# SuperbTUM/real-time-ReID-tracking

Hardware: AMD Instinct MI355X
Metric: crops/sec embedded + NxM distmat ms, ResNet18-SE 128x256 (higher is better)
Workload: dtype f16x3; 1 GPU; BASELINE configs[1]: ResNet18-SE embed 4096 distinct uint8 crops (128x256) per GPU + 4096x4096 L2 distmat; crops_per_gpu=4096, embed_dim=512, chunk=1024

## Files before the change

real-time-reid-tracking_amd/csrc/debug.hip:

```cpp
#include "reid_internal.h"
#include "pil_launch.h"
#include <string.h>
#include <stdlib.h>
#include <vector>

namespace {
struct Switch { const char* name; int reid_ctx::* field; };
const Switch kSwitches[] = {
    {"f16_cfg", &reid_ctx::f16_cfg}, {"f16_lin_256", &reid_ctx::f16_lin_256}, {"f16_split_k", &reid_ctx::f16_split_k},
    {"bank_fast", &reid_ctx::bank_fast}, {"side_copy", &reid_ctx::side_copy}, {"f32_stem_pool", &reid_ctx::f32_stem_pool},
    {"stem_split", &reid_ctx::stem_split}, {"split_pair", &reid_ctx::split_pair}, {"split_lean_epi", &reid_ctx::split_lean_epi},
    {"knn_wide", &reid_ctx::knn_wide}, {"f16_loader_prio", &reid_ctx::f16_loader_prio}, {"f16_frag_ahead", &reid_ctx::f16_frag_ahead},
    {"pack_epilogue", &reid_ctx::pack_epilogue}, {"f16_wide_splitk", &reid_ctx::f16_wide_splitk}, {"f32_split_k", &reid_ctx::f32_split_k},
    {"swin_fold", &reid_ctx::swin_fold}, {"swin_stop", &reid_ctx::swin_stop}, {"select_two_pass", &reid_ctx::select_two_pass},
    {"split_terms", &reid_ctx::split_terms}, {"f32_conv", &reid_ctx::f32_conv}, {"swin_attn_mfma", &reid_ctx::swin_attn_mfma},
    {"swin_attn_split", &reid_ctx::swin_attn_split}, {"swin_two_linear", &reid_ctx::swin_two_linear},
    {"f16_loader_waves", &reid_ctx::f16_loader_waves}, {"f16_halo", &reid_ctx::f16_halo}, {"f16_stem_fused", &reid_ctx::f16_stem_fused},
    {"f16_se_tail", &reid_ctx::f16_se_tail}, {"f16_c64", &reid_ctx::f16_c64}, {"swin_chunk_cap", &reid_ctx::swin_chunk_cap},
    {"split_x3", &reid_ctx::split_x3}, {"x3_ablate", &reid_ctx::x3_ablate}, {"x3_unroll", &reid_ctx::x3_unroll}, {"x3_narrow", &reid_ctx::x3_narrow}, {"conv_x3s", &reid_ctx::conv_x3s}, {"x3s_sk_cap", &reid_ctx::x3s_sk_cap}, {"x3_l4_narrow_nmt", &reid_ctx::x3_l4_narrow_nmt}, {"split_x3_small", &reid_ctx::split_x3_small}, {"split_x3_min_blocks", &reid_ctx::split_x3_min_blocks}, {"f32_dist_bk16", &reid_ctx::f32_dist_bk16}, {"lin_x3", &reid_ctx::lin_x3},
    {"host_pipeline", &reid_ctx::host_pipeline}, {"x3_sk_cap", &reid_ctx::x3_sk_cap}, {"chain", &reid_ctx::chain}, {"split_gemm_min_tiles", &reid_ctx::split_gemm_min_tiles},
    {"rerank_hbm_acc", &reid_ctx::rerank_hbm_acc}, {"gem_tail_min", &reid_ctx::gem_tail_min}, {"anysize_force", &reid_ctx::anysize_force},
};
}

extern "C" int reid_debug_set_switch(reid_ctx* ctx, const char* name, long long value) {
    ARG_CHECK(ctx && name);
    CTX_GUARD(ctx);
    HIP_TRY(hipStreamSynchronize(ctx->stream));
    if (!strcmp(name, "knn_wide_min")) {
        ctx->knn_wide_min = value;
        return REID_OK;
    }
    for (const Switch& s : kSwitches)
        if (!strcmp(name, s.name)) {
            if (!strcmp(name, "split_terms") && value != 3 && value != 4) break;
            ctx->*(s.field) = (int)value;
            return REID_OK;
        }
    reid_set_error("reid_debug_set_switch: no switch '%s' (or a value it does not take)", name);
    return REID_ERR_ARG;
}

extern "C" int reid_debug_get_switch(reid_ctx* ctx, const char* name, long long* value) {
    ARG_CHECK(ctx && name && value);
    if (!strcmp(name, "knn_wide_min")) {
        *value = ctx->knn_wide_min;
        return REID_OK;
    }
    for (const Switch& s : kSwitches)
        if (!strcmp(name, s.name)) {
            *value = ctx->*(s.field);
            return REID_OK;
        }
    reid_set_error("reid_debug_get_switch: no switch '%s'", name);
    return REID_ERR_ARG;
}

extern "C" int reid_debug_conv_f16(reid_ctx* ctx, int n, int h, int w, int cin, int cout, int r, int stride, int pad, int cfg,
                                   int iters, float* ms_per_launch) {
    ARG_CHECK(ctx && ms_per_launch && ctx->se18.loaded);
    CTX_GUARD(ctx);
    typedef _Float16 f16;
    const int ho = (h + 2 * pad - r) / stride + 1, wo = (w + 2 * pad - r) / stride + 1;
    const size_t nin = (size_t)n * h * w * cin, nw = (size_t)cout * r * r * cin, nout = (size_t)n * ho * wo * cout;
    f16 *x, *wt, *out;
    REID_TRY(ctx_ws(ctx, "dbg.x", nin * 2, (void**)&x));
    REID_TRY(ctx_ws(ctx, "dbg.w", nw * 2, (void**)&wt));
    REID_TRY(ctx_ws(ctx, "dbg.out", nout * 2, (void**)&out));
    const size_t src_n = ctx->se18.n_floats;
    for (size_t o = 0; o < nin; o += src_n) REID_TRY(launch_f32_to_f16(ctx, ctx->se18.blob, nin - o < src_n ? nin - o : src_n, x + o));
    for (size_t o = 0; o < nw; o += src_n) REID_TRY(launch_f32_to_f16(ctx, ctx->se18.blob, nw - o < src_n ? nw - o : src_n, wt + o));
    if (getenv("REID_DEBUG_ZERO")) {
        HIP_TRY(hipMemsetAsync(x, 0, nin * 2, ctx->stream));
        HIP_TRY(hipMemsetAsync(wt, 0, nw * 2, ctx->stream));
    }
    const int c0 = ctx->f16_cfg;
    const int h0 = ctx->f16_halo;
    ctx->f16_halo = cfg >= 2000000 ? 2 : 0;
    const int l0 = ctx->f16_loader_waves;
    if (cfg >= 2000000) ctx->f16_loader_waves = cfg & 1;
    ctx->f16_cfg = cfg >= 2000000 ? 0 : cfg;
    int st = REID_OK;
    for (int i = 0; i < 2 && st == REID_OK; ++i)
        st = conv_gemm16(ctx, A16_IM2COL, x, n, h, w, cin, wt, cout, r, r, stride, pad, r * r * cin, nullptr, nullptr, nullptr, 0, nullptr, out);
    if (st == REID_OK) st = reid_timer_start(ctx);
    for (int i = 0; i < iters && st == REID_OK; ++i)
        st = conv_gemm16(ctx, A16_IM2COL, x, n, h, w, cin, wt, cout, r, r, stride, pad, r * r * cin, nullptr, nullptr, nullptr, 0, nullptr, out);
    float ms = 0.f;
    if (st == REID_OK) st = reid_timer_stop(ctx, &ms);
    ctx->f16_cfg = c0;
    ctx->f16_halo = h0;
    ctx->f16_loader_waves = l0;
    *ms_per_launch = ms / (iters > 0 ? iters : 1);
    return st;
}


extern "C" int reid_debug_conv_split(reid_ctx* ctx, int n, int h, int w, int c, int cout, int ablate, int iters, float* ms_per_launch) {
    ARG_CHECK(ctx && ms_per_launch && ctx->se18.loaded && c % 64 == 0 && cout % 64 == 0);
    CTX_GUARD(ctx);
    typedef _Float16 f16;
    const size_t nin = (size_t)n * h * w * 2 * c, nw = (size_t)cout * 9 * 3 * c, nout = (size_t)n * h * w * cout;
    f16 *x, *wt;
    float *out, *sc;
    REID_TRY(ctx_ws(ctx, "dbgs.x", nin * 2, (void**)&x));
    REID_TRY(ctx_ws(ctx, "dbgs.w", nw * 2, (void**)&wt));
    REID_TRY(ctx_ws(ctx, "dbgs.out", nout * 4, (void**)&out));
    REID_TRY(ctx_ws(ctx, "dbgs.sc", (size_t)cout * 2 * 4, (void**)&sc));
    const size_t src_n = ctx->se18.n_floats;
    for (size_t o = 0; o < nin; o += src_n) REID_TRY(launch_f32_to_f16(ctx, ctx->se18.blob, nin - o < src_n ? nin - o : src_n, x + o));
    for (size_t o = 0; o < nw; o += src_n) REID_TRY(launch_f32_to_f16(ctx, ctx->se18.blob, nw - o < src_n ? nw - o : src_n, wt + o));
    HIP_TRY(hipMemcpyAsync(sc, ctx->se18.blob, (size_t)cout * 2 * 4, hipMemcpyDeviceToDevice, ctx->stream));
    if (ablate & 128) {
        HIP_TRY(hipMemsetAsync(x, 0, nin * 2, ctx->stream));
        HIP_TRY(hipMemsetAsync(wt, 0, nw * 2, ctx->stream));
    }
    Gemm16Params q;
    memset(&q, 0, sizeof(q));
    q.split_terms = 3;
    q.H = h; q.W = w; q.Cin = 3 * c; q.R = 3; q.S = 3; q.stride = 1; q.pad = 1; q.Ho = h; q.Wo = w;
    q.M = n * h * w; q.N = cout; q.K = 27 * c; q.ldb = q.K;
    q.A = x; q.B = wt; q.C32 = out; q.ldc = cout;
    q.col_scale = sc; q.col_shift = sc + cout; q.relu = 1;
    q.acc_scale = 1.0f / 2048.0f;
    q.zero_page = ctx->se18.zero_page;
    q.ablate = ablate & 127;
    q.diag = ctx->conv_diag;
    int st = REID_OK;
    for (int i = 0; i < 2 && st == REID_OK; ++i) st = launch_conv3x3_split(ctx, q, REID_K_CONV_GEMM, 0, 0);
    if (st == REID_OK) st = reid_timer_start(ctx);
    for (int i = 0; i < iters && st == REID_OK; ++i) st = launch_conv3x3_split(ctx, q, REID_K_CONV_GEMM, 0, 0);
    float ms = 0.f;
    if (st == REID_OK) st = reid_timer_stop(ctx, &ms);
    *ms_per_launch = ms / (iters > 0 ? iters : 1);
    return st;
}

extern "C" int reid_debug_conv_c64(reid_ctx* ctx, int n, const float* x, const float* w_krsc, const float* scale,
                                   const float* shift, const float* residual, int relu, float* out, float* stats) {
    ARG_CHECK(ctx && x && w_krsc && out && n >= 1);
    CTX_GUARD(ctx);
    typedef _Float16 f16;
    const size_t nact = (size_t)n * 64 * 32 * 64, nw = 64 * 576;
    float *xf, *wf, *rf = nullptr, *sc = nullptr, *sh = nullptr, *st = nullptr, *of;
    f16 *xh, *wh, *rh = nullptr, *oh, *zp;
    REID_TRY(ctx_ws(ctx, "dbg64.xf", nact * 4, (void**)&xf));
    REID_TRY(ctx_ws(ctx, "dbg64.wf", nw * 4, (void**)&wf));
    REID_TRY(ctx_ws(ctx, "dbg64.xh", nact * 2, (void**)&xh));
    REID_TRY(ctx_ws(ctx, "dbg64.wh", nw * 2, (void**)&wh));
    REID_TRY(ctx_ws(ctx, "dbg64.oh", nact * 2, (void**)&oh));
    REID_TRY(ctx_ws(ctx, "dbg64.of", nact * 4, (void**)&of));
    REID_TRY(ctx_ws(ctx, "dbg64.zp", 256, (void**)&zp));
    REID_TRY(ctx_ws(ctx, "dbg64.sc", 64 * 4, (void**)&sc));
    REID_TRY(ctx_ws(ctx, "dbg64.sh", 64 * 4, (void**)&sh));
    REID_TRY(ctx_ws(ctx, "dbg64.st", (size_t)n * 128 * 4, (void**)&st));
    HIP_TRY(hipMemsetAsync(zp, 0, 256, ctx->stream));
    HIP_TRY(hipMemcpyAsync(xf, x, nact * 4, hipMemcpyHostToDevice, ctx->stream));
    HIP_TRY(hipMemcpyAsync(wf, w_krsc, nw * 4, hipMemcpyHostToDevice, ctx->stream));
    std::vector<float> ones(64, 1.f);
    HIP_TRY(hipMemcpyAsync(sc, scale ? scale : ones.data(), 64 * 4, hipMemcpyHostToDevice, ctx->stream));
    if (shift) HIP_TRY(hipMemcpyAsync(sh, shift, 64 * 4, hipMemcpyHostToDevice, ctx->stream));
    REID_TRY(launch_f32_to_f16(ctx, xf, nact, xh));
    REID_TRY(launch_scale_rows_f16(ctx, wf, sc, 64, 576, wh));
    if (residual) {
        REID_TRY(ctx_ws(ctx, "dbg64.rf", nact * 4, (void**)&rf));
        REID_TRY(ctx_ws(ctx, "dbg64.rh", nact * 2, (void**)&rh));
        HIP_TRY(hipMemcpyAsync(rf, residual, nact * 4, hipMemcpyHostToDevice, ctx->stream));
        REID_TRY(launch_f32_to_f16(ctx, rf, nact, rh));
    }
    HIP_TRY(hipStreamSynchronize(ctx->stream));
    REID_TRY(launch_conv3x3_c64_f16(ctx, xh, n, wh, shift ? sh : nullptr, rh, relu, stats ? st : nullptr, oh, zp));
    std::vector<f16> tmp(nact);
    HIP_TRY(hipMemcpyAsync(tmp.data(), oh, nact * 2, hipMemcpyDeviceToHost, ctx->stream));
    if (stats) HIP_TRY(hipMemcpyAsync(stats, st, (size_t)n * 128 * 4, hipMemcpyDeviceToHost, ctx->stream));
// ... 1253 lines not shown
```

real-time-reid-tracking_amd/csrc/reid_internal.h:

```cpp
#pragma once
#include <hip/hip_runtime.h>
#include <stdint.h>
#include <stddef.h>
#include <stdio.h>
#include <initializer_list>
#include <string>
#include <map>
#include <tuple>
#include <vector>
#include "../../include/reid_hip.h"
struct reid_ctx;

void reid_set_error(const char* fmt, ...);

#define HIP_TRY(expr)                                                                         \
    do {                                                                                      \
        hipError_t _e = (expr);                                                               \
        if (_e != hipSuccess) {                                                               \
            reid_set_error("%s:%d %s -> %s", __FILE__, __LINE__, #expr, hipGetErrorString(_e)); \
            return REID_ERR_HIP;                                                              \
        }                                                                                     \
    } while (0)

#define REID_TRY(expr)            \
// ... 202 lines not shown
int launch_scale_rows_f16(reid_ctx*, const float* w, const float* scale, int rows, int k, _Float16* out);
int launch_conv3x3_c64_f16(reid_ctx*, const _Float16* in, int n, const _Float16* w_scaled, const float* shift,
                           const _Float16* residual, int relu, float* stats, _Float16* out, const _Float16* zero_page,
                           const float* se_w1 = nullptr, const float* se_w2t = nullptr);
int launch_stem_w16_scaled(reid_ctx*, const float* stem_w_f32, const float* scale, _Float16* out);
int launch_stem_pool_f16(reid_ctx*, const _Float16* pad_in, const uint8_t* crops_u8, int n, const _Float16* w16s, const float* shift,
                         _Float16* pooled);
int launch_conv_w16_chunked(reid_ctx*, const float* w_f32, int cout, int rs, int cin, _Float16* out);
int launch_gemm_f32(reid_ctx* ctx, int amode, int epi, const GemmParams& p, int kind, double flops, double bytes);
int launch_ta_tail(reid_ctx* ctx, const float* y, const float* sc, int n_img, int H, int W, int C, const float* wts, float* out);
int launch_ema_tail(reid_ctx* ctx, const float* y, const float* sc, int n_img, int H, int W, int C, const float* prm, float* out);
int launch_stem_split(reid_ctx* ctx, const void* x, bool is_u8, int n, const float* wgt, const float* scale, const float* shift, float* out,
                      _Float16* packed);
int launch_stem_f32(reid_ctx* ctx, const void* x, bool is_u8, int n, const float* wgt, const float* scale, const float* shift,
                    float* out, bool pooled);
bool gemm_f32_dma_supported(int amode, int epi, const GemmParams& p);
int launch_gemm_f32_dma(reid_ctx* ctx, int epi, const GemmParams& p, int kind, double flops, double bytes);
bool conv_f32_supported(const GemmParams& p);
int launch_conv_f32(reid_ctx* ctx, const GemmParams& p, int kind, double flops, double bytes);
bool conv_f32_general_supported(const GemmParams& p);
int launch_conv_f32_general(reid_ctx* ctx, const GemmParams& p, int kind, double flops, double bytes);

int launch_nchw_to_nhwc3(reid_ctx*, const float* x_nchw, int n, int h, int w, float* out_nhwc);
int launch_resize_norm(reid_ctx*, const uint8_t* packed, const long long* offsets, const int* hw, int n, int H, int W,
                       int pitch, float* out_nhwc);
int launch_maxpool3s2(reid_ctx*, const float* x, int n, int h, int w, int c, float* out);
int launch_norm_finalize(reid_ctx*, const float* stats, int n_img, int tiles, int c, int half, int hw,
                         const float* in_gamma, const float* in_beta, const float* bn_scale, const float* bn_shift,
                         float* a_scale, float* a_shift);
int launch_in_apply(reid_ctx*, float* x, const float* stats, int n_img, int tiles, int c, int half, int hw, const float* in_gamma,
                    const float* in_beta);
int launch_se_finalize(reid_ctx*, const float* stats, int n_img, int tiles, int c, int mid, int hw, const float* w1,
                       const float* w2, float* s);
int tail_slices(int n_img, int hw);
int launch_se_tail(reid_ctx*, const float* stats, int n_img, int tiles, int c, int mid, int hw, const float* w1, const float* w2,
                   const float* y, const float* sc, float* out, _Float16* packed = nullptr);
int launch_se_tail_form(reid_ctx*, int form, const float* stats, int n_img, int tiles, int c, int mid, int hw, const float* w1,
                        const float* w2, const float* y, const float* sc, float* out, _Float16* packed);
int launch_se_combine(reid_ctx*, const float* y, const float* sc, const float* s, int n_img, int hw, int c, float* out);
int launch_in_apply_pack(reid_ctx*, const float* x, const float* stats, int n_img, int tiles, int c, int half, int hw,
                         const float* in_gamma, const float* in_beta, _Float16* packed,
                         bool in_half_only = false);
int launch_gem_neck(reid_ctx*, const float* x, int n_img, int hw, int c, const float* p, const float* scale,
                    const float* shift, float* gem_out, float* emb);
int launch_gem_neck_tail(reid_ctx*, const float* stats, int n_img, int tiles, int c, int mid, int hw, const float* w1, const float* w2,
                         const float* y, const float* sc, const float* p, const float* scale, const float* shift, float* gem_out,
                         float* emb);
int launch_row_sqnorm(reid_ctx*, const float* x, int m, int d, long long ld, float* out);
int launch_argmin_rows(reid_ctx*, const float* dist, int m, int n, long long ld, int32_t* idx, float* val);
int launch_topk_rows(reid_ctx*, const float* dist, int m, int n, long long ld, int k, float* D, int32_t* I);
int launch_rank_eval(reid_ctx*, const float* score, int nq, int ng, long long ld, const long long* ql,
                     const long long* qc, const long long* gl, const long long* gc, int32_t* cmc_sum, double* ap,
                     int32_t* valid);
int launch_diou_cost(reid_ctx*, const double* tracks, int t, const double* dets, int m, double* out, int as_cost);

struct ProfSlot {
    double ms = 0, flops = 0, bytes = 0;
    long long launches = 0;
};

struct Se18Block {
    int c, cin, stride, ibn, ds, mid;
    const float *conv1_w, *in_gamma, *in_beta, *bn1_scale, *bn1_shift, *conv2_w, *bn2_scale, *bn2_shift;
    const float *ds_w, *ds_scale, *ds_shift, *se_w1, *se_w2;
    const float *ta, *ema;
};

struct Se18Weights {
    bool loaded = false;
    float* blob = nullptr;
    size_t n_floats = 0;
    int num_class = 0;
    int arch = 0;
    const float *stem_w, *stem_scale, *stem_shift;
    Se18Block blk[8];
    const float *gem_p, *neck_scale, *neck_shift, *cls_w;
    const float* cam_bias = nullptr;
    int num_cams = 0;
    float cam_factor = -1.0f;
    _Float16* blob16 = nullptr;
    _Float16* stem_w16 = nullptr;
    _Float16* l1_conv2_w16s[2] = {nullptr, nullptr};
    _Float16* stem_w16s = nullptr;
    _Float16* zero_page = nullptr;
    float* ep = nullptr;
    const _Float16* h(const float* p) const { return blob16 + (p - blob); }
};

struct reid_comm_loop {
    virtual int allgather(int rank, const void* d_send, void* d_recv, size_t bytes, hipStream_t st) = 0;
    virtual int allreduce(int rank, double* inout, int count, int op) = 0;
    virtual void detach(int rank) = 0;
    virtual ~reid_comm_loop() {}
};
struct reid_comm {
    void* comm = nullptr;
    int rank = 0, world = 1;
    reid_comm_loop* loop = nullptr;
};
void comm_release(reid_ctx* ctx);
int launch_knn_merge(reid_ctx* ctx, const float* Dall, const int32_t* Iall, int world, int nq, int kk, int k, float* D, int32_t* I);

struct reid_ctx {
    int device = 0;
    reid_comm* comm = nullptr;
    hipStream_t stream = nullptr;
    hipStream_t own_stream = nullptr;
    int chunk = 1024;
    int precision = 0;
    bool profile = false;
    ProfSlot prof[REID_K_COUNT];
    std::vector<std::pair<hipEvent_t, hipEvent_t>> ev_pool;
    struct Pending { int kind; hipEvent_t a, b; double flops, bytes; };
    std::vector<Pending> pending;
    hipEvent_t t0 = nullptr, t1 = nullptr;
    std::map<std::string, std::pair<void*, size_t>> ws;
    std::map<std::string, std::pair<void*, size_t>> pinned;
    std::map<const void*, void*> split_w;
    int bank_fast = 1;
    Se18Weights se18;
    int last_n = 0;
    int swin_last_n = 0, swin_last_tok = 0;
    int debug_keep = 0;
    bool last_f16 = false;
    int f16_wide_splitk = 1;
    int f16_frag_ahead = 1;
    int f16_loader_prio = 1;
    int f16_loader_waves = 1;
    int f16_halo = 1;
    int gem_tail_min = 120;
    int f16_se_tail = 1;
    int f16_c64 = 2;
    int f16_stem_fused = 2;
    int f32_conv = 1;
    int f32_split_k = 1;
    int lin_x3 = 1;
    int f32_dist_bk16 = 1;
    int pack_epilogue = 1;
    int split_lean_epi = 1;
    int split_x3 = 3;
    int split_gemm_min_tiles = 128;
    int chain = 0;
    int x3_sk_cap = 0;
    int split_x3_small = 2;
    int x3s_sk_cap = 8;
    int conv_x3s = 1;
    int x3_l4_narrow_nmt = 31;
    int x3_narrow = 1;
    int x3_unroll = 3;
    int x3_ablate = 0;
    int split_x3_min_blocks = 512;
    int split_pair = 0;
    int stem_split = 1;
    int f32_stem_pool = 1;
    int split_terms = 3;
    int knn_wide = 1;
    long long knn_wide_min = 1ll << 25;
    int knn_wide_force = 0;
    int select_exp = 0;
    int select_two_pass = 0;
    int rerank_hbm_acc = 0;
    int swin_stop = -1;
    int swin_fold = 1;
    int swin_two_linear = 1;
    int swin_attn_split = 0;
    int two_linear_ablate = 0;
    int swin_attn_mfma = 1;
    int f16_split_k = 1;
    int swin_chunk_cap = 1024;
    int f16_lin_256 = 1;
    int f16_cfg = 0;
    int frame_m[2] = {0, 0};
    float* frame_emb[2] = {nullptr, nullptr};
    int frame_d[2] = {512, 512};
    int frame_pending[2] = {0, 0}, frame_has[2] = {0, 0};
    size_t frame_tm[2] = {0, 0};
    hipEvent_t frame_ev[2] = {nullptr, nullptr};
    hipStream_t match_stream = nullptr;
    int match_async = 0;
    hipEvent_t join_ev = nullptr;
    hipEvent_t fwd_ev[2] = {nullptr, nullptr}, match_ev[2] = {nullptr, nullptr};
    hipStream_t copy_stream = nullptr;
    hipEvent_t copy_ev = nullptr;
    std::vector<hipEvent_t> pipe_ev;
    int host_pipeline = 1;
    int side_copy = 1;
    std::vector<int32_t> side_idx;
    size_t side_cursor = 0;
    const char* frame_out[2] = {nullptr, nullptr};
    float* stage_ptr[11] = {nullptr};
    size_t stage_elems[11] = {0};
    int anysize_force = 0;
    unsigned long long* conv_diag = nullptr;
    int conv_form = 0;
    std::string split_bad_se18, split_bad_swin;
    int* fault = nullptr;
};
enum { REID_FAULT_RANGE = 1, REID_FAULT_NONFINITE = 2 };
int ctx_fault_status(reid_ctx* ctx);
bool knn_wide_eligible(reid_ctx* ctx, int nq, int nb, int d, int k);
int knn_wide_dev(reid_ctx* ctx, const float* xp, int nq, const float* yp, int nb, int ld, const float* rs, const float* cq, int k, float* d_D,
                 int32_t* d_I);

inline std::string split_range_violation(const float* blob, const std::map<std::string, std::pair<size_t, size_t>>& tab,
                                         const std::vector<std::pair<std::string, float>>& suffix_bound) {
    for (const auto& kv : tab) {
        for (const auto& sb : suffix_bound) {
            const std::string& suf = sb.first;
            if (kv.first.size() < suf.size() || kv.first.compare(kv.first.size() - suf.size(), suf.size(), suf) != 0) continue;
            float mx = 0.f;
            const float* w = blob + kv.second.first;
            for (size_t i = 0; i < kv.second.second; ++i) {
                const float a = w[i] < 0 ? -w[i] : w[i];
                if (!(a <= mx)) mx = a;
            }
            if (!(mx < sb.second)) {
                char buf[160];
                snprintf(buf, sizeof(buf), "%s (max |w| = %g, limit %g)", kv.first.c_str(), (double)mx, (double)sb.second);
                return buf;
            }
            break;
        }
    }
    return std::string();
}

struct ChainElem {
    const float* x;
    const float* stats;
    const float* sc;
    const float *g, *b;
    float* out;
    _Float16* packed;
    int c, half, hw, tiles, mid, slices;
};
struct ChainStage {
    int kind;
    int idx;
    int first, items;
    int dep;
    int target;
    int sk;
};
struct ChainParams {
    int n_img, n_stages, total_items, flags;
    ChainStage st[8];
    Gemm16Params conv[4];
    ChainElem el[4];
    int* counters;
    int* fault;
};
int launch_chain(reid_ctx* ctx, const ChainParams& cp, int W);

int conv_gemm(reid_ctx* ctx, int amode, const void* x, int n, int H, int W, int Cin, const float* wgt, int Cout, int R,
              int S, int stride, int pad, int Kpad, const float* a_scale, const float* a_shift, int a_relu,
              const float* col_scale, const float* col_shift, const float* residual, int relu, float* stats, float* out,
              int relu_from = 0, const _Float16* x_packed = nullptr,
              _Float16* out_packed = nullptr, int pack_from = 0, bool* packed_written = nullptr);
int conv_weights_fresh(reid_ctx* ctx, const float* d_w);
int conv_weights_splittable(reid_ctx* ctx, const float* h_w, size_t count, const char* who);
int conv_gemm16(reid_ctx* ctx, int amode, const _Float16* x, int n, int H, int W, int Cin, const _Float16* wgt, int Cout,
                int R, int S, int stride, int pad, int K, const float* col_scale, const float* col_shift,
                const _Float16* residual, int relu, float* stats, _Float16* out, int Hp = 0, int Wp = 0);

struct DeviceGuard {
    int prev = -1, dev = -1;
    explicit DeviceGuard(int d) : dev(d) {
        if (hipGetDevice(&prev) != hipSuccess) prev = -1;
        if (prev != dev) (void)hipSetDevice(dev);
    }
    ~DeviceGuard() {
        if (prev >= 0 && prev != dev) (void)hipSetDevice(prev);
    }
    DeviceGuard(const DeviceGuard&) = delete;
    DeviceGuard& operator=(const DeviceGuard&) = delete;
};
#define CTX_GUARD(ctx) DeviceGuard _dev_guard((ctx)->device)
#define CTX_ENTER(ctx)            \
    CTX_GUARD(ctx);               \
    REID_TRY(ctx_fault_status(ctx))

void swin_release(reid_ctx* ctx);
int ctx_ws(reid_ctx* ctx, const char* name, size_t bytes, void** out);
int ctx_take_side(reid_ctx* ctx, int n, int rows, const char* what, const int32_t** d_idx);
int launch_add_indexed_rows(reid_ctx* ctx, float* x, int n, long long hw, int C, const float* table, const int32_t* d_idx, float coeff);
int ctx_pinned(reid_ctx* ctx, const char* name, size_t bytes, void** out);
int ctx_pipe_events(reid_ctx* ctx, int passes);

template <class Up, class Run, class Down>
int host_passes(reid_ctx* ctx, int n, int pass, Up up, Run run, Down down) {
    const int passes = (n + pass - 1) / pass;
    if (passes <= 1 || !ctx->host_pipeline) {
        REID_TRY(up(0, n, ctx->stream));
        for (int i = 0; i < n; i += pass) REID_TRY(run(i, n - i < pass ? n - i : pass));
        REID_TRY(down(0, n, ctx->stream));
        HIP_TRY(hipStreamSynchronize(ctx->stream));
        return REID_OK;
    }
    REID_TRY(ctx_pipe_events(ctx, passes));
    hipStream_t cs = ctx->copy_stream;
    hipEvent_t* up_ev = ctx->pipe_ev.data();
    hipEvent_t* run_ev = ctx->pipe_ev.data() + passes;
    auto span = [&](int k, int* i, int* m) { *i = k * pass; *m = n - *i < pass ? n - *i : pass; };
    int i, m, rc = REID_OK;
    span(0, &i, &m);
    rc = up(i, m, cs);
// ... 111 lines not shown
```

real-time-reid-tracking_amd/csrc/stem_split.hip:

```cpp
#include "reid_internal.h"

typedef _Float16 f16;
typedef f16 half8 __attribute__((ext_vector_type(8)));
typedef float f32x16 __attribute__((ext_vector_type(16)));
typedef unsigned int u32x2 __attribute__((ext_vector_type(2)));

namespace {

constexpr int IMG_H = 256, IMG_W = 128, OUT_H = 128, OUT_W = 64;
constexpr int PITCH = 144 * 8;
constexpr int RING = 32;
constexpr int WROW = 14 * 32 + 16;

__device__ __forceinline__ unsigned split_pair(float x) {
    const f16 h = (f16)x;
    const f16 l = (f16)((x - (float)h) * 2048.0f);
    return (unsigned)__builtin_bit_cast(unsigned short, h) | ((unsigned)__builtin_bit_cast(unsigned short, l) << 16);
}

template <bool U8>
__global__ __launch_bounds__(512, 1) void stem_split_kernel(const void* __restrict__ x, const float* __restrict__ wgt,
                                                            const float* __restrict__ scale, const float* __restrict__ shift,
                                                            int nseg, float* __restrict__ out, f16* __restrict__ packed,
                                                            int* __restrict__ fault) {
    extern __shared__ __attribute__((aligned(16))) unsigned char smem[];
    unsigned char* const img_h = smem;
    unsigned char* const img_l = img_h + RING * PITCH;
    unsigned char* const w_h = img_l + RING * PITCH;
    unsigned char* const w_l = w_h + 64 * WROW;
    float* const edge = (float*)(w_l + 64 * WROW);

    const int tid = threadIdx.x, lane = tid & 63, wave = tid >> 6;
    const int li = lane & 31, lh = lane >> 5;
    const int cw = wave & 3, cb = wave >> 2;
    const int img = blockIdx.x / nseg, seg = blockIdx.x - img * nseg;
    const int t0 = seg * (OUT_H / 2) / nseg, t1 = (seg + 1) * (OUT_H / 2) / nseg;

    for (int i = tid; i < 2 * RING * PITCH / 16; i += 512) ((uint4*)smem)[i] = uint4{0u, 0u, 0u, 0u};
    __syncthreads();
    for (int i = tid; i < 64 * 14 * 16; i += 512) {
        const int n = i / 224, k = i - n * 224, s = k >> 4, h = (k >> 3) & 1, j = k & 7;
        const int px = 2 * (2 * (s & 1) + h) + (j >> 2), c = j & 3;
        const float v = (px < 7 && c < 3) ? wgt[n * 192 + (s >> 1) * 24 + px * 3 + c] : 0.f;
        const unsigned hl = split_pair(v);
        *(unsigned short*)(w_h + n * WROW + k * 2) = (unsigned short)hl;
        *(unsigned short*)(w_l + n * WROW + k * 2) = (unsigned short)(hl >> 16);
        if constexpr (U8) {
            const float wh = (float)__builtin_bit_cast(f16, (unsigned short)hl), wl = (float)__builtin_bit_cast(f16, (unsigned short)(hl >> 16));
            const f16 ll = (f16)(((v - wh) * 2048.0f - wl) * 2048.0f);
            *(unsigned short*)(img_l + n * WROW + k * 2) = __builtin_bit_cast(unsigned short, ll);
        }
    }
    __syncthreads();

    const int f_row = tid >> 7, f_px = tid & 127;
    const int f_off = (3 * f_px) & ~3, f_off2 = f_off + 4 < IMG_W * 3 ? f_off + 4 : f_off, f_sh = 8 * ((3 * f_px) & 3);
    auto fetch = [&](int j, unsigned (&raw)[3]) __attribute__((always_inline)) {
        const int iy = 4 * j + 2 + f_row;
        raw[0] = raw[1] = raw[2] = 0u;
        if ((unsigned)iy < (unsigned)IMG_H) {
            if constexpr (U8) {
                const uint8_t* p = (const uint8_t*)x + ((long long)img * IMG_H + iy) * (IMG_W * 3);
                raw[0] = *(const unsigned*)(p + f_off);
                raw[1] = *(const unsigned*)(p + f_off2);
            } else {
                const float* p = (const float*)x + (((long long)img * IMG_H + iy) * IMG_W + f_px) * 3;
                raw[0] = __float_as_uint(p[0]); raw[1] = __float_as_uint(p[1]); raw[2] = __float_as_uint(p[2]);
            }
        }
    };
    auto commit = [&](int j, const unsigned (&raw)[3]) __attribute__((always_inline)) {
        const int iy = 4 * j + 2 + f_row;
        unsigned a = 0u, b = 0u, c = 0u;
        const int at = ((iy - 2) & (RING - 1)) * PITCH + (3 + f_px) * 8;
        if constexpr (U8) {
            if ((unsigned)iy < (unsigned)IMG_H) {
                const unsigned px = (unsigned)((((unsigned long long)raw[1] << 32) | raw[0]) >> f_sh);
                a = __builtin_bit_cast(unsigned short, (f16)(float)(2 * (int)(px & 0xffu) - 255));
                b = __builtin_bit_cast(unsigned short, (f16)(float)(2 * (int)((px >> 8) & 0xffu) - 255));
                c = __builtin_bit_cast(unsigned short, (f16)(float)(2 * (int)((px >> 16) & 0xffu) - 255));
            }
            *(u32x2*)(img_h + at) = u32x2{a | (b << 16), c};
            return;
        }
        if ((unsigned)iy < (unsigned)IMG_H) {
            a = split_pair(__uint_as_float(raw[0])); b = split_pair(__uint_as_float(raw[1])); c = split_pair(__uint_as_float(raw[2]));
        }
        *(u32x2*)(img_h + at) = u32x2{(a & 0xffffu) | (b << 16), c & 0xffffu};
        *(u32x2*)(img_l + at) = u32x2{(a >> 16) | (b & 0xffff0000u), c >> 16};
    };

    const int ox = cw * 16 + (li & 15);
    const int a_col = (2 * ox + 2 * lh) * 8;
    const int b_at = (cb * 32 + li) * WROW + lh * 16;
    const float cs = U8 ? scale[cb * 32 + li] / 255.0f : scale[cb * 32 + li], sh = shift[cb * 32 + li];

    const int t_first = t0 > 0 ? t0 - 1 : t0;
    const int ntile = t1 - t_first;
    float prev[8], pend = 0.f;
#pragma unroll
    for (int e = 0; e < 8; ++e) prev[e] = -INFINITY;
    float* const pool_img = out + (long long)img * (OUT_H / 2) * (OUT_W / 2) * 64;
    f16* const pack_img = packed ? packed + (long long)img * (OUT_H / 2) * (OUT_W / 2) * 128 : nullptr;
    unsigned vmag = 0u;
    auto store = [&](int t, int col, float v) __attribute__((always_inline)) {
        const long long pix = (long long)t * (OUT_W / 2) + col;
        pool_img[pix * 64 + cb * 32 + li] = v;
        if (pack_img) {
            vmag = range_acc(vmag, v);
            const unsigned hl = split_pair(v);
            *(unsigned short*)(pack_img + pix * 128 + cb * 32 + li) = (unsigned short)hl;
            *(unsigned short*)(pack_img + pix * 128 + 64 + cb * 32 + li) = (unsigned short)(hl >> 16);
        }
    };
    auto finish_first_column = [&](int t) __attribute__((always_inline)) {
        if (cw > 0 && lh == 0) store(t, cw * 8, fmaxf(pend, edge[((t & 1) * 4 + cw - 1) * 64 + cb * 32 + li]));
    };

    unsigned raw_a[3], raw_b[3];
    for (int j = t_first - 2; j <= t_first + 1; ++j) {
        fetch(j, raw_a);
        commit(j, raw_a);
    }
    const int t_last = t_first + ntile - 1;
    fetch(t_first + 2, raw_a);
    __syncthreads();
    auto mma = [&](int t) __attribute__((always_inline)) -> f32x16 {
        f32x16 acc, cor, cor2;
#pragma unroll
        for (int e = 0; e < 16; ++e) acc[e] = cor[e] = cor2[e] = 0.f;
        const int row0 = 4 * t - 5 + 2 * (li >> 4);
        half8 av[3], alv[3], bhv[3], blv[3];
        auto load_step = [&](int st, int buf) __attribute__((always_inline)) {
            const int a_at = ((row0 + (st >> 1)) & (RING - 1)) * PITCH + a_col + 32 * (st & 1);
            av[buf] = *(const half8*)(img_h + a_at);
            bhv[buf] = *(const half8*)(w_h + b_at + 32 * st);
            blv[buf] = *(const half8*)(w_l + b_at + 32 * st);
            if constexpr (U8) alv[buf] = *(const half8*)(img_l + b_at + 32 * st);
            else alv[buf] = *(const half8*)(img_l + a_at);
        };
        load_step(0, 0);
        load_step(1, 1);
#pragma unroll
        for (int st = 0; st < 14; ++st) {
            const int buf = st % 3;
            if (st + 2 < 14) load_step(st + 2, (st + 2) % 3);
            __builtin_amdgcn_sched_barrier(0);
            acc = __builtin_amdgcn_mfma_f32_32x32x16_f16(av[buf], bhv[buf], acc, 0, 0, 0);
            if constexpr (U8) cor2 = __builtin_amdgcn_mfma_f32_32x32x16_f16(av[buf], alv[buf], cor2, 0, 0, 0);
            else cor = __builtin_amdgcn_mfma_f32_32x32x16_f16(alv[buf], bhv[buf], cor, 0, 0, 0);
            cor = __builtin_amdgcn_mfma_f32_32x32x16_f16(av[buf], blv[buf], cor, 0, 0, 0);
            __builtin_amdgcn_sched_barrier(0);
        }
        constexpr float S1 = 1.0f / 2048.0f;
        f32x16 v;
#pragma unroll
        for (int e = 0; e < 16; ++e) v[e] = (acc[e] + (cor[e] + cor2[e] * S1) * S1) * cs + sh;
        return v;
    };
    auto epilogue = [&](int t, const f32x16 v) __attribute__((always_inline)) {
        const bool emit = t >= t0;
        if (emit && t > t_first && t > t0) finish_first_column(t - 1);
        float vm[8];
#pragma unroll
        for (int e = 0; e < 8; ++e) {
            vm[e] = fmaxf(fmaxf(prev[e], v[e]), v[e + 8]);
            prev[e] = v[e + 8];
        }
        if (emit) {
            const float m01 = fmaxf(vm[0], vm[1]), m45 = fmaxf(vm[4], vm[5]);
            const float pa = fmaxf(fmaxf(vm[1], vm[2]), vm[3]), pb = fmaxf(fmaxf(vm[5], vm[6]), vm[7]);
            const float s0 = lh ? m01 : vm[3], s1 = lh ? vm[3] : m45, s2 = lh ? m45 : vm[7];
            const float p2 = fmaxf(s0, __shfl_xor(s0, 32)), p4 = fmaxf(s1, __shfl_xor(s1, 32)), p6 = fmaxf(s2, __shfl_xor(s2, 32));
            store(t, cw * 8 + 1 + 2 * lh, pa);
            store(t, cw * 8 + 5 + 2 * lh, pb);
            store(t, cw * 8 + (lh ? 4 : 2), lh ? p4 : p2);
            if (lh) {
                store(t, cw * 8 + 6, p6);
                edge[((t & 1) * 4 + cw) * 64 + cb * 32 + li] = vm[7];
            } else if (cw == 0) {
                store(t, 0, m01);
            } else {
                pend = m01;
            }
        }
    };
    const bool defer = cb == 1;
    f32x16 vkeep;
#pragma unroll
    for (int e = 0; e < 16; ++e) vkeep[e] = 0.f;
    auto tile = [&](int t, unsigned (&raw_commit)[3], unsigned (&raw_fetch)[3]) __attribute__((always_inline)) {
        if (t + 3 <= t_last) fetch(t + 3, raw_fetch);
        if (defer) {
            if (t > t_first) epilogue(t - 1, vkeep);
            vkeep = mma(t);
        } else {
            vkeep = mma(t);
        }
        if (t + 2 <= t_last) commit(t + 2, raw_commit);
        if (!defer) epilogue(t, vkeep);
        __syncthreads();
    };
    for (int t = t_first; t <= t_last; t += 2) {
        tile(t, raw_a, raw_b);
        if (t + 1 <= t_last) tile(t + 1, raw_b, raw_a);
    }
    if (defer) epilogue(t_last, vkeep);
    __syncthreads();
    finish_first_column(t1 - 1);
    range_raise(fault, vmag);
}

constexpr int SMEM = 2 * RING * PITCH + 2 * 64 * WROW + 2 * 4 * 64 * 4;

}

int launch_stem_split(reid_ctx* ctx, const void* x, bool is_u8, int n, const float* wgt, const float* scale, const float* shift, float* out,
                      _Float16* packed) {
    ARG_CHECK(n >= 1);
    int nseg = 1;
    if (n < 256) {
        long long best = -1;
        for (int s = 1; s <= 64; ++s) {
            const long long rounds = ((long long)n * s + 255) / 256;
            const long long cost = rounds * (3 + 5 * ((64 + s - 1) / s + (s > 1 ? 1 : 0)));
            if (best < 0 || cost < best) { best = cost; nseg = s; }
        }
    }
    const int grid = n * nseg;
    if (is_u8) HIP_TRY(hipFuncSetAttribute((const void*)stem_split_kernel<true>, hipFuncAttributeMaxDynamicSharedMemorySize, SMEM));
    else HIP_TRY(hipFuncSetAttribute((const void*)stem_split_kernel<false>, hipFuncAttributeMaxDynamicSharedMemorySize, SMEM));
    const double flops = 2.0 * n * OUT_H * OUT_W * 64 * 147.0;
    const double bytes = (double)n * IMG_H * IMG_W * 3 * (is_u8 ? 1.0 : 4.0) + (double)n * OUT_H * OUT_W * 64 * (packed ? 2.0 : 1.0) + 64 * 147 * 4.0;
    prof_begin(ctx, REID_K_CONV_GEMM, flops, bytes);
    if (is_u8) hipLaunchKernelGGL((stem_split_kernel<true>), dim3(grid), dim3(512), SMEM, ctx->stream, x, wgt, scale, shift, nseg, out, packed,
                                  ctx->fault);
    else hipLaunchKernelGGL((stem_split_kernel<false>), dim3(grid), dim3(512), SMEM, ctx->stream, x, wgt, scale, shift, nseg, out, packed, ctx->fault);
    prof_end(ctx);
    LAUNCH_CHECK();
    return REID_OK;
}
```

Baseline: 85240 crops/s.

## Make stem conv kernel persistent, walking images per block with prefetch overlap

For large batches the stem conv+pool kernel now launches one block per compute unit, and each block loops over images with a grid stride instead of using one block per image. The first rows of the next image are prefetched while the current image's epilogue finishes, and weight staging into shared memory is paid once per block rather than once per image. The epilogue is also restructured to use precomputed byte offsets and permlane32_swap in place of shuffles, and the wave index is made uniform with readfirstlane. The risk is load imbalance when the image count does not divide evenly by the CU count, and the loss of overlap between independent blocks.

```diff
diff --git a/real-time-reid-tracking_amd/csrc/debug.hip b/real-time-reid-tracking_amd/csrc/debug.hip
--- a/real-time-reid-tracking_amd/csrc/debug.hip
+++ b/real-time-reid-tracking_amd/csrc/debug.hip
@@ -20,6 +20,7 @@
     {"split_x3", &reid_ctx::split_x3}, {"x3_ablate", &reid_ctx::x3_ablate}, {"x3_unroll", &reid_ctx::x3_unroll}, {"x3_narrow", &reid_ctx::x3_narrow}, {"conv_x3s", &reid_ctx::conv_x3s}, {"x3s_sk_cap", &reid_ctx::x3s_sk_cap}, {"x3_l4_narrow_nmt", &reid_ctx::x3_l4_narrow_nmt}, {"split_x3_small", &reid_ctx::split_x3_small}, {"split_x3_min_blocks", &reid_ctx::split_x3_min_blocks}, {"f32_dist_bk16", &reid_ctx::f32_dist_bk16}, {"lin_x3", &reid_ctx::lin_x3},
     {"host_pipeline", &reid_ctx::host_pipeline}, {"x3_sk_cap", &reid_ctx::x3_sk_cap}, {"chain", &reid_ctx::chain}, {"split_gemm_min_tiles", &reid_ctx::split_gemm_min_tiles},
     {"rerank_hbm_acc", &reid_ctx::rerank_hbm_acc}, {"gem_tail_min", &reid_ctx::gem_tail_min}, {"anysize_force", &reid_ctx::anysize_force},
+    {"stem_walk_min", &reid_ctx::stem_walk_min}, {"stem_walk_blocks", &reid_ctx::stem_walk_blocks},
 };
 }
 
diff --git a/real-time-reid-tracking_amd/csrc/reid_internal.h b/real-time-reid-tracking_amd/csrc/reid_internal.h
--- a/real-time-reid-tracking_amd/csrc/reid_internal.h
+++ b/real-time-reid-tracking_amd/csrc/reid_internal.h
@@ -378,6 +378,8 @@
     int split_x3_min_blocks = 512;
     int split_pair = 0;
     int stem_split = 1;
+    int stem_walk_min = 256;
+    int stem_walk_blocks = 0;
     int f32_stem_pool = 1;
     int split_terms = 3;
     int knn_wide = 1;
diff --git a/real-time-reid-tracking_amd/csrc/stem_split.hip b/real-time-reid-tracking_amd/csrc/stem_split.hip
--- a/real-time-reid-tracking_amd/csrc/stem_split.hip
+++ b/real-time-reid-tracking_amd/csrc/stem_split.hip
@@ -30,11 +30,15 @@
     unsigned char* const w_l = w_h + 64 * WROW;
     float* const edge = (float*)(w_l + 64 * WROW);
 
-    const int tid = threadIdx.x, lane = tid & 63, wave = tid >> 6;
+    const int tid = threadIdx.x, lane = tid & 63, wave = __builtin_amdgcn_readfirstlane(tid >> 6);
     const int li = lane & 31, lh = lane >> 5;
     const int cw = wave & 3, cb = wave >> 2;
-    const int img = blockIdx.x / nseg, seg = blockIdx.x - img * nseg;
-    const int t0 = seg * (OUT_H / 2) / nseg, t1 = (seg + 1) * (OUT_H / 2) / nseg;
+    const bool walk = nseg < 0;
+    int img = walk ? (int)blockIdx.x : (int)blockIdx.x / nseg;
+    const int img_end = walk ? -nseg : img + 1, img_step = walk ? (int)gridDim.x : 1;
+    const int seg = walk ? 0 : (int)blockIdx.x - img * nseg, nstrip = walk ? 1 : nseg;
+    const int t0 = seg * (OUT_H / 2) / nstrip, t1 = (seg + 1) * (OUT_H / 2) / nstrip;
+    if (img >= img_end) return;
 
     for (int i = tid; i < 2 * RING * PITCH / 16; i += 512) ((uint4*)smem)[i] = uint4{0u, 0u, 0u, 0u};
     __syncthreads();
@@ -98,33 +102,34 @@
     const int t_first = t0 > 0 ? t0 - 1 : t0;
     const int ntile = t1 - t_first;
     float prev[8], pend = 0.f;
-#pragma unroll
-    for (int e = 0; e < 8; ++e) prev[e] = -INFINITY;
-    float* const pool_img = out + (long long)img * (OUT_H / 2) * (OUT_W / 2) * 64;
-    f16* const pack_img = packed ? packed + (long long)img * (OUT_H / 2) * (OUT_W / 2) * 128 : nullptr;
+    char *pool_img = nullptr, *pack_img = nullptr;
+    const unsigned ch = cb * 32 + li;
+    const unsigned col_a = cw * 8 + 1 + 2 * lh, col_c = cw * 8 + (lh ? 4 : 2), col_d = cw * 8 + (lh ? 6 : 0);
+    const unsigned o32_a = col_a * 256 + ch * 4, o32_c = col_c * 256 + ch * 4, o32_d = col_d * 256 + ch * 4;
+    const unsigned o16_a = col_a * 256 + ch * 2, o16_c = col_c * 256 + ch * 2, o16_d = col_d * 256 + ch * 2;
+    float* const edge_w = edge + cw * 64 + ch;
+    const float* const edge_r = edge + (cw > 0 ? cw - 1 : 0) * 64 + ch;
     unsigned vmag = 0u;
-    auto store = [&](int t, int col, float v) __attribute__((always_inline)) {
-        const long long pix = (long long)t * (OUT_W / 2) + col;
-        pool_img[pix * 64 + cb * 32 + li] = v;
+    auto put = [&](int t, unsigned o32, unsigned o16, int add, float v) __attribute__((always_inline)) {
+        *(float*)(pool_img + (size_t)t * 8192 + add + (size_t)o32) = v;
         if (pack_img) {
             vmag = range_acc(vmag, v);
             const unsigned hl = split_pair(v);
-            *(unsigned short*)(pack_img + pix * 128 + cb * 32 + li) = (unsigned short)hl;
-            *(unsigned short*)(pack_img + pix * 128 + 64 + cb * 32 + li) = (unsigned short)(hl >> 16);
-        }
-    };
-    auto finish_first_column = [&](int t) __attribute__((always_inline)) {
-        if (cw > 0 && lh == 0) store(t, cw * 8, fmaxf(pend, edge[((t & 1) * 4 + cw - 1) * 64 + cb * 32 + li]));
-    };
-
-    unsigned raw_a[3], raw_b[3];
-    for (int j = t_first - 2; j <= t_first + 1; ++j) {
-        fetch(j, raw_a);
-        commit(j, raw_a);
-    }
+            char* const p = pack_img + (size_t)t * 8192 + add + (size_t)o16;
+            *(unsigned short*)p = (unsigned short)hl;
+            *(unsigned short*)(p + 128) = (unsigned short)(hl >> 16);
+        }
+    };
+    auto finish_fourth = [&](int t) __attribute__((always_inline)) {
+        if (cw > 0) put(t, o32_d, o16_d, 0, lh ? pend : fmaxf(pend, edge_r[(t & 1) * 256]));
+    };
+
+    unsigned raw_a[3], raw_b[3], raw4[4][3];
     const int t_last = t_first + ntile - 1;
-    fetch(t_first + 2, raw_a);
-    __syncthreads();
+    auto fetch4 = [&]() __attribute__((always_inline)) {
+#pragma unroll
+        for (int k = 0; k < 4; ++k) fetch(t_first - 2 + k, raw4[k]);
+    };
     auto mma = [&](int t) __attribute__((always_inline)) -> f32x16 {
         f32x16 acc, cor, cor2;
 #pragma unroll
@@ -159,31 +164,27 @@
         return v;
     };
     auto epilogue = [&](int t, const f32x16 v) __attribute__((always_inline)) {
-        const bool emit = t >= t0;
-        if (emit && t > t_first && t > t0) finish_first_column(t - 1);
+        if (t > t0 && t > t_first) finish_fourth(t - 1);
         float vm[8];
 #pragma unroll
         for (int e = 0; e < 8; ++e) {
             vm[e] = fmaxf(fmaxf(prev[e], v[e]), v[e + 8]);
             prev[e] = v[e + 8];
         }
-        if (emit) {
-            const float m01 = fmaxf(vm[0], vm[1]), m45 = fmaxf(vm[4], vm[5]);
-            const float pa = fmaxf(fmaxf(vm[1], vm[2]), vm[3]), pb = fmaxf(fmaxf(vm[5], vm[6]), vm[7]);
-            const float s0 = lh ? m01 : vm[3], s1 = lh ? vm[3] : m45, s2 = lh ? m45 : vm[7];
-            const float p2 = fmaxf(s0, __shfl_xor(s0, 32)), p4 = fmaxf(s1, __shfl_xor(s1, 32)), p6 = fmaxf(s2, __shfl_xor(s2, 32));
-            store(t, cw * 8 + 1 + 2 * lh, pa);
-            store(t, cw * 8 + 5 + 2 * lh, pb);
-            store(t, cw * 8 + (lh ? 4 : 2), lh ? p4 : p2);
-            if (lh) {
-                store(t, cw * 8 + 6, p6);
-                edge[((t & 1) * 4 + cw) * 64 + cb * 32 + li] = vm[7];
-            } else if (cw == 0) {
-                store(t, 0, m01);
-            } else {
-                pend = m01;
-            }
-        }
+        if (t < t0) return;
+        const float m01 = fmaxf(vm[0], vm[1]), m45 = fmaxf(vm[4], vm[5]);
+        const float pa = fmaxf(fmaxf(vm[1], vm[2]), vm[3]), pb = fmaxf(fmaxf(vm[5], vm[6]), vm[7]);
+        const auto x0 = __builtin_amdgcn_permlane32_swap(__float_as_uint(m01), __float_as_uint(m45), false, false);
+        const auto x1 = __builtin_amdgcn_permlane32_swap(__float_as_uint(vm[7]), __float_as_uint(vm[7]), false, false);
+        const float p24 = fmaxf(vm[3], __uint_as_float(lh ? x0[0] : x0[1]));
+        const float p6 = fmaxf(m45, __uint_as_float(x1[0]));
+        put(t, o32_a, o16_a, 0, pa);
+        put(t, o32_a, o16_a, 4 * 256, pb);
+        put(t, o32_c, o16_c, 0, p24);
+        if (lh) edge_w[(t & 1) * 256] = vm[7];
+        const float fourth = lh ? p6 : m01;
+        if (cw == 0) put(t, o32_d, o16_d, 0, fourth);
+        else pend = fourth;
     };
     const bool defer = cb == 1;
     f32x16 vkeep;
@@ -201,13 +202,28 @@
         if (!defer) epilogue(t, vkeep);
         __syncthreads();
     };
-    for (int t = t_first; t <= t_last; t += 2) {
-        tile(t, raw_a, raw_b);
-        if (t + 1 <= t_last) tile(t + 1, raw_b, raw_a);
-    }
-    if (defer) epilogue(t_last, vkeep);
-    __syncthreads();
-    finish_first_column(t1 - 1);
+    fetch4();
+    for (;;) {
+#pragma unroll
+        for (int k = 0; k < 4; ++k) commit(t_first - 2 + k, raw4[k]);
+        fetch(t_first + 2, raw_a);
+        pool_img = (char*)out + (size_t)img * ((OUT_H / 2) * (OUT_W / 2) * 64 * 4);
+        pack_img = packed ? (char*)packed + (size_t)img * ((OUT_H / 2) * (OUT_W / 2) * 128 * 2) : nullptr;
+#pragma unroll
+        for (int e = 0; e < 8; ++e) prev[e] = -INFINITY;
+        __syncthreads();
+        for (int t = t_first; t <= t_last; t += 2) {
+            tile(t, raw_a, raw_b);
+            if (t + 1 <= t_last) tile(t + 1, raw_b, raw_a);
+        }
+        img += img_step;
+        const bool more = img < img_end;
+        if (more) fetch4();
+        if (defer) epilogue(t_last, vkeep);
+        __syncthreads();
+        finish_fourth(t1 - 1);
+        if (!more) break;
+    }
     range_raise(fault, vmag);
 }
 
@@ -227,7 +243,13 @@
             if (best < 0 || cost < best) { best = cost; nseg = s; }
         }
     }
-    const int grid = n * nseg;
+    int grid = n * nseg;
+    if (n >= ctx->stem_walk_min) {
+        int blocks = ctx->stem_walk_blocks;
+        if (blocks <= 0) HIP_TRY(hipDeviceGetAttribute(&blocks, hipDeviceAttributeMultiprocessorCount, ctx->device));
+        grid = n < blocks ? n : blocks;
+        nseg = -n;
+    }
     if (is_u8) HIP_TRY(hipFuncSetAttribute((const void*)stem_split_kernel<true>, hipFuncAttributeMaxDynamicSharedMemorySize, SMEM));
     else HIP_TRY(hipFuncSetAttribute((const void*)stem_split_kernel<false>, hipFuncAttributeMaxDynamicSharedMemorySize, SMEM));
     const double flops = 2.0 * n * OUT_H * OUT_W * 64 * 147.0;
```

New measurement: 85420 crops/s (median of 6 runs). No clear change (+0.2%).
